# HalfSummer11/CAPTRA

Hardware: AMD Instinct MI355X
Metric: tracked frames/sec (4096-pt clouds) (higher is better)
Workload: dtype f32; 1 GPU; NOCS-REAL275-shaped rigid category 'bottle' (1 part, symmetric), 4096 pts/frame, batch=32 trajectories per GPU, fp32 (BASELINE.json configs[1]); points=4096, trajectories_per_gpu=32, distinct_clouds_per_gpu=32, parallelism=dp1 (trajectory-sharded, RCCL all-gather of poses), weights=seeded default_rng(7), real architecture (3.96 M params), physical-regime plants

## Files before the change

captra_amd/csrc/sa_pipe.hip:

```cpp
#include "wave_mlp.h"

namespace {

constexpr int SP_POS = 128;

struct SpParams {
    int b, n, m, k;
    const float *v1pm;
    const float *xyz_cn;
    const float *new_xyz;
    const int *idx;
    const float *w1;
    const float *w2, *b2, *w3, *b3;
    float *out;
    int out_ctotal, co_off;
    unsigned long long *prof;
    int split;
    int *dyn;
};

#define SP_TICK(slot)                                                           \
    if (CAPTRA_PROF_ON(p.prof)) {                                                    \
        const unsigned long long t_now = __builtin_amdgcn_s_memtime();          \
        if (lane == 0 && sampled) atomicAdd(p.prof + (slot), t_now - t_last);   \
        t_last = t_now;                                                         \
    }

template <int NOUT>
__device__ __forceinline__ void sp_mid_unit(const f32x16 &acc, int t, int q, float (&hout)[NOUT]) {
    unsigned a[4];
#pragma unroll
    for (int i = 0; i < 4; ++i) {
        const int x = __float_as_int(acc[4 * q + i]);
        a[i] = (unsigned)(x > 0 ? x : 0);
    }
    const auto p01 = __builtin_amdgcn_permlane32_swap(a[0], a[1], false, false);
    const auto p23 = __builtin_amdgcn_permlane32_swap(a[2], a[3], false, false);
    const int k0 = 16 * t + 4 * q;
    if (k0 + 0 < NOUT) hout[k0 + 0] = __uint_as_float(p01[0]);
    if (k0 + 1 < NOUT) hout[k0 + 1] = __uint_as_float(p23[0]);
    if (k0 + 2 < NOUT) hout[k0 + 2] = __uint_as_float(p01[1]);
    if (k0 + 3 < NOUT) hout[k0 + 3] = __uint_as_float(p23[1]);
}

struct SpMaxState {
    int w[8];
    int u[2];
};

__device__ __forceinline__ void sp_max_stage_a(const f32x16 &acc, SpMaxState &st, int lane) {
    const bool b0 = lane & 1;
#pragma unroll
    for (int i = 0; i < 8; ++i) {
        const int x0 = __float_as_int(acc[2 * i]), x1 = __float_as_int(acc[2 * i + 1]);
        const int own = b0 ? x1 : x0, oth = b0 ? x0 : x1;
        st.w[i] = imax_dpp<0xB1>(own, oth);
    }
}

__device__ __forceinline__ void sp_max_stage_bc(SpMaxState &st, int lane) {
    const bool b1 = lane & 2, b2 = lane & 4;
    int v[4];
#pragma unroll
    for (int j = 0; j < 4; ++j) {
        const int own = b1 ? st.w[2 * j + 1] : st.w[2 * j], oth = b1 ? st.w[2 * j] : st.w[2 * j + 1];
        v[j] = imax_dpp<0x4E>(own, oth);
    }
#pragma unroll
    for (int m = 0; m < 2; ++m) {
        const int own = b2 ? v[2 * m + 1] : v[2 * m], oth = b2 ? v[2 * m] : v[2 * m + 1];
        const int p = dpp_keep<0x104, 0xF, 0x5>(own, oth);
        const int q = dpp_keep<0x114, 0xF, 0xA>(p, oth);
        st.u[m] = imax(own, q);
    }
}

__device__ __forceinline__ void sp_max_stage_d(const SpMaxState &st, int &zr) {
    const int lane = (int)(threadIdx.x & 63);
    const bool b3 = lane & 8;
    const int own = b3 ? st.u[1] : st.u[0], oth = b3 ? st.u[0] : st.u[1];
    zr = imax(zr, imax_dpp<0x128>(own, oth));
}

template <int COUT, bool LAST, int NPARTS, int NOUT, int NZ>
__device__ __forceinline__ void sp_epi_part(const f32x16 (&acc)[2], int ps, int c, float (&hout)[NOUT], int (&zrun)[NZ],
                                            SpMaxState (&mst)[2], int lane) {
    constexpr int NT = (COUT + 31) / 32;
    if constexpr (LAST) {
#pragma unroll
        for (int u = 0; u < 6; ++u)
            if (u * NPARTS / 6 == c && 2 * ps + u / 3 < NT) {
                const int tm = u / 3;
                if (u % 3 == 0) sp_max_stage_a(acc[tm], mst[tm], lane);
                else if (u % 3 == 1) sp_max_stage_bc(mst[tm], lane);
                else sp_max_stage_d(mst[tm], zrun[2 * ps + tm < NZ ? 2 * ps + tm : 0]);
            }
    } else {
#pragma unroll
        for (int u = 0; u < 8; ++u)
            if (u * NPARTS / 8 == c && 2 * ps + (u >> 2) < NT) sp_mid_unit<NOUT>(acc[u >> 2], 2 * ps + (u >> 2), u & 3, hout);
    }
}


template <int CIN, int COUT, bool LAST, int START, int NIN, int NOUT, int NZ, typename Next, typename Side>
__device__ __forceinline__ void sp_layer(const float *wt, const float *bias_lds, const float (&hin)[NIN], float (&hout)[NOUT],
                                         float (&s)[3][16], int (&zrun)[NZ], int lane, Next next, Side side) {
    using S = SwShape<CIN, COUT>;
    static_assert(NIN >= S::KST, "input operand array too small");
    const __amdgpu_buffer_rsrc_t rsrc = sw_frag_rsrc<CIN, COUT>(wt);
    const int voff = lane * 16;
    f32x16 acc[2][2];
    SpMaxState mst[2];
    static_assert(!LAST || S::NSETS >= 6 || S::NPASS == 1, "the deferred max needs its six units in distinct steps, in order");
#pragma unroll
    for (int g = 0; g < S::STEPS; ++g) {
        const int ps = g / S::NSETS, c = g % S::NSETS, pb = ps & 1;
        if (c == 0) {
#pragma unroll
            for (int tm = 0; tm < 2; ++tm)
                if (2 * ps + tm < S::NT) sw_bias_init(acc[pb][tm], bias_lds, 2 * ps + tm, lane);
        }
        if (g == 0 && S::STEPS > 1) sw_load_set<CIN, COUT>(s[(START + 1) % 3], rsrc, voff, 1 / S::NSETS, 1 % S::NSETS);
        if (g + 2 < S::STEPS) sw_load_set<CIN, COUT>(s[(START + g + 2) % 3], rsrc, voff, (g + 2) / S::NSETS, (g + 2) % S::NSETS);
        if (g + 2 == S::STEPS || (S::STEPS == 1 && g == 0)) next(s[(START + S::STEPS) % 3]);
        side(g);
        __builtin_amdgcn_sched_barrier(0);
#pragma unroll
        for (int j = 0; j < SW_KS; ++j)
#pragma unroll
            for (int tm = 0; tm < 2; ++tm) {
                const int kk = c * SW_KS + j;
                if (kk < S::KST && 2 * ps + tm < S::NT)
                    acc[pb][tm] = __builtin_amdgcn_mfma_f32_32x32x2f32(s[(START + g) % 3][tm * SW_KS + j], hin[kk], acc[pb][tm], 0, 0, 0);
            }
        if (ps > 0) {
            sp_epi_part<COUT, LAST, S::NSETS>(acc[pb ^ 1], ps - 1, c, hout, zrun, mst, lane);
#pragma unroll
            for (int i = 0; i < 2 * SW_KS; ++i) {
                __builtin_amdgcn_sched_group_barrier(0x008, 1, 0);
                __builtin_amdgcn_sched_group_barrier(0x002, 4, 0);
            }
        }
        __builtin_amdgcn_sched_barrier(0);
    }
    constexpr int LP = S::NPASS - 1;
#pragma unroll
    for (int c = 0; c < S::NSETS; ++c) sp_epi_part<COUT, LAST, S::NSETS>(acc[LP & 1], LP, c, hout, zrun, mst, lane);
}

template <int CF, int C1, int C2, int C3>
__device__ __forceinline__ void sp_body(const SpParams &p, const int blk, const int nblk) {
    using S1 = SwShape<CF + 3, C1>;
    using S2 = SwShape<C1, C2>;
    using S3 = SwShape<C2, C3>;
    constexpr int NT1 = S1::NT;
    static_assert(NT1 <= 4 && C1 % 32 == 0, "first-layer width");
    __shared__ __attribute__((aligned(16))) float bias_lds[2 * 256];
    const int tid = threadIdx.x, lane = tid & 63, half = lane >> 5;
    const int wave = __builtin_amdgcn_readfirstlane(tid >> 6);

    for (int e = tid; e < 2 * 256; e += 256) {
        const int c = e & 255;
        bias_lds[e] = e < 256 ? (c < pad128c(C2) ? p.b2[c] : 0.f) : (c < pad128c(C3) ? p.b3[c] : 0.f);
    }
    float at[2][NT1];
    {
        const __amdgpu_buffer_rsrc_t rw = __builtin_amdgcn_make_buffer_rsrc((void *)p.w1, 0, S1::KP * S1::LDW * 4, 0x00020000);
        const int voff_w = (half * S1::LDW + (lane & 31)) * 4;
#pragma unroll
        for (int jj = 0; jj < 2; ++jj)
#pragma unroll
            for (int t = 0; t < NT1; ++t)
                at[jj][t] = __builtin_bit_cast(float, __builtin_amdgcn_raw_buffer_load_b32(rw, voff_w, ((CF + 2 * jj) * S1::LDW + 32 * t) * 4, 0));
    }
    __syncthreads();

    const int nwaves = nblk * 4, gid = blk * 4 + wave;
    const int ncentres = p.b * p.m;
    const int nslices = p.k / 32;
    int id = 0;
    float bt[2] = {0.f, 0.f};
    float4 g4[NT1][4];
    auto load_id = [&](int c, int sl) { return p.idx[(size_t)c * p.k + sl * 32 + (lane & 31)]; };
    auto load_rest = [&](int c, int id_, float (&bt_)[2], float4 (&g_)[NT1][4]) {
        const int tb = c / p.m;
        const float *cp = p.new_xyz + (size_t)c * 3;
#pragma unroll
        for (int jj = 0; jj < 2; ++jj) {
            const int a = 2 * jj + half;
            bt_[jj] = a < 3 ? p.xyz_cn[((size_t)tb * 3 + a) * p.n + id_] - cp[a] : 0.f;
        }
        const float4 *vp = reinterpret_cast<const float4 *>(p.v1pm + ((size_t)tb * p.n + id_) * C1 + 4 * half);
#pragma unroll
        for (int t = 0; t < NT1; ++t)
#pragma unroll
            for (int q = 0; q < 4; ++q) g_[t][q] = vp[8 * t + 2 * q];
    };

    const bool sampled = blk % 16 == 0;
    unsigned long long t_last = CAPTRA_PROF_ON(p.prof) ? __builtin_amdgcn_s_memtime() : 0ull;
    float s[3][16];
    constexpr int START3 = S2::STEPS % 3;
    constexpr int NEXT2 = (START3 + S3::STEPS) % 3;
    int zrun[S3::NT];
    const bool split = p.split != 0;
    const int ssh = __builtin_ctz((unsigned)nslices);
    int task = gid;
    int c = split ? gid >> ssh : gid, sl = split ? gid & (nslices - 1) : 0;
    const bool dyn = p.dyn != nullptr && !split && nslices > 1;
    int dyn_raw = 0, c_next = gid + nwaves;
    if (dyn) {
        if (lane == 0) dyn_raw = atomicAdd(p.dyn, 1);
        c = __builtin_amdgcn_readfirstlane(dyn_raw);
    }
    if (c < ncentres) {
        sw_first_set<C1, C2>(s[NEXT2], p.w2, lane);
        id = load_id(c, sl);
        load_rest(c, id, bt, g4);
    }
    while (c < ncentres) {
        if (sl == 0 || split) {
#pragma unroll
            for (int t = 0; t < S3::NT; ++t) zrun[t] = 0;
        }
        const bool last_slice = split || sl + 1 == nslices;
        if (dyn) {
            if (sl == 0 && lane == 0) dyn_raw = atomicAdd(p.dyn, 1);
            if (last_slice) c_next = __builtin_amdgcn_readfirstlane(dyn_raw);
        } else {
            c_next = c + nwaves;
        }
        const int cn = split ? (task + nwaves) >> ssh : (last_slice ? c_next : c), sn = split ? (task + nwaves) & (nslices - 1) : (last_slice ? 0 : sl + 1);
        const bool has_next = cn < ncentres;
        int id_n = 0;

        float h1[S2::KST], h2[S3::KST], none[1];
        SP_TICK(0)
        if (NEXT2 != 0) {
#pragma unroll
            for (int i = 0; i < 16; ++i) s[0][i] = s[NEXT2][i];
        }
        {
            f32x16 acc[NT1];
#pragma unroll
            for (int t = 0; t < NT1; ++t)
#pragma unroll
                for (int q = 0; q < 4; ++q) {
                    acc[t][4 * q + 0] = g4[t][q].x; acc[t][4 * q + 1] = g4[t][q].y;
                    acc[t][4 * q + 2] = g4[t][q].z; acc[t][4 * q + 3] = g4[t][q].w;
                }
#pragma unroll
            for (int jj = 0; jj < 2; ++jj)
#pragma unroll
                for (int t = 0; t < NT1; ++t) acc[t] = __builtin_amdgcn_mfma_f32_32x32x2f32(at[jj][t], bt[jj], acc[t], 0, 0, 0);
#pragma unroll
            for (int t = 0; t < NT1; ++t) sw_mid_epilogue<S2::KST>(acc[t], t, h1);
        }
        __builtin_amdgcn_sched_barrier(0);
        SP_TICK(1)
        sp_layer<C1, C2, false, 0>(p.w2, bias_lds, h1, h2, s, zrun, lane,
                                   [&](float (&dst)[16]) { sw_first_set<C2, C3>(dst, p.w3, lane); },
                                   [&](int g) { if (g == 1 && has_next) id_n = load_id(cn, sn); });
        SP_TICK(2)
        sp_layer<C2, C3, true, START3>(p.w3, bias_lds + 256, h2, none, s, zrun, lane,
                                       [&](float (&dst)[16]) { sw_first_set<C1, C2>(dst, p.w2, lane); },
                                       [&](int g) { if (g == 2 && has_next) load_rest(cn, id_n, bt, g4); });
        id = id_n;
        SP_TICK(3)
        if (CAPTRA_PROF_ON(p.prof) && lane == 0 && sampled) atomicAdd(p.prof + 9, 1ull);
        if (last_slice) {
            const int tb = c / p.m, centre = c - tb * p.m;
            const int r = lane & 15;
            const int row0 = 8 * (r >> 2) + (r & 3) + 4 * half;
            float *op = p.out + ((size_t)tb * p.out_ctotal + p.co_off + row0) * p.m + centre;
#pragma unroll
            for (int t = 0; t < S3::NT; ++t) {
                const float v = sw_bfly_finish(zrun[t]);
                if ((lane & 16) == 0 && 32 * t + row0 < C3) {
                    if (split) atomicMax(reinterpret_cast<int *>(op + (size_t)32 * t * p.m), __float_as_int(v));
                    else op[(size_t)32 * t * p.m] = v;
                }
            }
            SP_TICK(4)
        }
        c = cn; sl = sn; task += nwaves;
    }
}


template <int CF, int C1, int C2, int C3>
__global__ __launch_bounds__(256) __attribute__((amdgpu_waves_per_eu(1, 1))) void sa_wave_pipe_kernel(SpParams p) {
    sp_body<CF, C1, C2, C3>(p, (int)blockIdx.x, (int)gridDim.x);
}

struct Sp2Params { SpParams s[2]; int g0; };
__global__ __launch_bounds__(256) __attribute__((amdgpu_waves_per_eu(1, 1))) void sa_wave_pipe2_kernel(Sp2Params q) {
    const int blk = (int)blockIdx.x;
    if (blk < q.g0) sp_body<320, 128, 128, 256>(q.s[0], blk, q.g0);
    else sp_body<320, 128, 196, 256>(q.s[1], blk - q.g0, (int)gridDim.x - q.g0);
}

}

extern unsigned long long *captra_sa_prof_ptr();
extern int captra_sa_split_knob();
extern int *captra_sa_dyn_slot(const captra_launch_opts *o, hipStream_t stream);

struct SpRecord { SpParams q; unsigned grid; int code; };
struct SpCollect { SpRecord rec[2]; int n; };
void captra_sp_collect_init(void *buf, size_t bytes) {
    static_assert(sizeof(SpCollect) <= 1024, "SlCollect::sp (sa_fused.hip) holds an SpCollect");
    if (buf != nullptr && bytes >= sizeof(SpCollect)) static_cast<SpCollect *>(buf)->n = 0;
}
int captra_sp_collect_flush(void *buf, hipStream_t s) {
    SpCollect &c = *static_cast<SpCollect *>(buf);
    const int n = c.n;
    c.n = 0;
    if (n == 2 && c.rec[0].code == 0 && c.rec[1].code == 1 && c.rec[0].q.dyn == nullptr && c.rec[1].q.dyn == nullptr) {
        Sp2Params q2;
        q2.s[0] = c.rec[0].q; q2.s[1] = c.rec[1].q; q2.g0 = (int)c.rec[0].grid;
        CAPTRA_LAUNCH("sa_scale_fused", sa_wave_pipe2_kernel, dim3(c.rec[0].grid + c.rec[1].grid), dim3(256), 0, s, q2);
        return captra_last_error();
    }
    for (int i = 0; i < n; ++i) {
        if (c.rec[i].code == 0) { CAPTRA_LAUNCH("sa_scale_fused", (sa_wave_pipe_kernel<320, 128, 128, 256>), dim3(c.rec[i].grid), dim3(256), 0, s, c.rec[i].q); }
        else { CAPTRA_LAUNCH("sa_scale_fused", (sa_wave_pipe_kernel<320, 128, 196, 256>), dim3(c.rec[i].grid), dim3(256), 0, s, c.rec[i].q); }
    }
    return captra_last_error();
}

int captra_sa_scale_pre_pm_impl(int b, int n, int m, int k, int cfeat, int c1, int c2, int c3, const float *v1pm,
                                const float *xyz_cn, const float *new_xyz, const int *idx, const float *w1,
                                const float *w2, const float *b2, const float *w3, const float *b3, float *out,
                                int out_ctotal, int co_off, const captra_launch_opts *opts, void *spbuf, captra_stream_t stream) {
    SpCollect *col = static_cast<SpCollect *>(spbuf);
    if (b < 0 || n < 1 || m < 0 || k < 1 || cfeat < 1 || c1 < 1 || c2 < 1 || c3 < 1 || v1pm == nullptr) return -1;
    if (out_ctotal < co_off + c3 || co_off < 0) return -1;
    if (k % 32 != 0 || 128 % k != 0) return -2;
    const long long L = (long long)m * k;
    if (L % SP_POS != 0 || (long long)c1 * n * 4 >= (1ll << 31) || (long long)b * L >= (1ll << 31)) return -2;
    if (b == 0 || m == 0) return 0;
    SpParams q;
    q.b = b; q.n = n; q.m = m; q.k = k; q.v1pm = v1pm; q.xyz_cn = xyz_cn; q.new_xyz = new_xyz; q.idx = idx;
    q.w1 = w1; q.w2 = w2; q.b2 = b2; q.w3 = w3; q.b3 = b3; q.out = out; q.out_ctotal = out_ctotal; q.co_off = co_off;
    q.prof = captra_sa_prof_ptr();
    const int cus = captra_free_cus(opts);
    const long long centres = (long long)b * m;
    if (centres >= (1ll << 30)) return -2;
    const int split_knob = captra_sa_split_knob();
    q.split = (split_knob != 0 && k > 32 && (split_knob == 2 || centres < 4ll * cus)) ? 1 : 0;
    const long long wgs = ((q.split ? centres * (k / 32) : centres) + 3) / 4;
    const unsigned grid = (unsigned)(wgs < cus ? wgs : cus);
    q.dyn = (!q.split && k > 32 && wgs > 1 && col == nullptr) ? captra_sa_dyn_slot(opts, (hipStream_t)stream) : nullptr;
    if (q.split && !(opts != nullptr && opts->sa_prezeroed)) {
        if (b <= 8 && ((size_t)c3 * m * 4) % 16 == 0 && (reinterpret_cast<uintptr_t>(out + (size_t)co_off * m) & 15) == 0 && ((size_t)out_ctotal * m * 4) % 16 == 0) {
            for (int bb = 0; bb < b; ++bb) (void)captra_zero_async(out + ((size_t)bb * out_ctotal + co_off) * m, (size_t)c3 * m * 4, (hipStream_t)stream);
        } else {
            (void)hipMemset2DAsync(out + (size_t)co_off * m, (size_t)out_ctotal * m * 4, 0, (size_t)c3 * m * 4, b, (hipStream_t)stream);
        }
    }
#define SPP_CASE(CF_, C1_, C2_, C3_)                                                                                  \
    if (cfeat == CF_ && c1 == C1_ && c2 == C2_ && c3 == C3_) {                                                        \
        auto kern = sa_wave_pipe_kernel<CF_, C1_, C2_, C3_>;                                                          \
        if (col != nullptr && col->n < 2) {                                                                           \
            col->rec[col->n].q = q; col->rec[col->n].grid = grid; col->rec[col->n].code = (C2_ == 128 ? 0 : 1);       \
            ++col->n;                                                                                                 \
            return 0;                                                                                                 \
        }                                                                                                             \
        CAPTRA_LAUNCH("sa_scale_fused", kern, dim3(grid), dim3(256), 0, (hipStream_t)stream, q);                       \
        return captra_last_error();                                                                                   \
    }
    SPP_CASE(320, 128, 128, 256)
    SPP_CASE(320, 128, 196, 256)
#undef SPP_CASE
    return -2;
}

extern "C" int captra_sa_scale_pre_pm_ex(int b, int n, int m, int k, int cfeat, int c1, int c2, int c3, const float *v1pm,
                                         const float *xyz_cn, const float *new_xyz, const int *idx, const float *w1,
                                         const float *w2, const float *b2, const float *w3, const float *b3, float *out,
                                         int out_ctotal, int co_off, const captra_launch_opts *opts, captra_stream_t stream) {
    return captra_sa_scale_pre_pm_impl(b, n, m, k, cfeat, c1, c2, c3, v1pm, xyz_cn, new_xyz, idx, w1, w2, b2, w3, b3, out, out_ctotal, co_off, opts, nullptr, stream);
}
extern "C" int captra_sa_scale_pre_pm(int b, int n, int m, int k, int cfeat, int c1, int c2, int c3, const float *v1pm,
                                      const float *xyz_cn, const float *new_xyz, const int *idx, const float *w1,
                                      const float *w2, const float *b2, const float *w3, const float *b3, float *out,
                                      int out_ctotal, int co_off, captra_stream_t stream) {
    return captra_sa_scale_pre_pm_impl(b, n, m, k, cfeat, c1, c2, c3, v1pm, xyz_cn, new_xyz, idx, w1, w2, b2, w3, b3, out, out_ctotal, co_off, nullptr, nullptr, stream);
}
```

Before: 5891 frames/s.

## Compute layer-2 remainder channels with VALU FMAs instead of an extra MFMA tile

When the second MLP layer width leaves four channels past a multiple of 32, those four channels are now computed with scalar FMAs. Their weights are staged in LDS and h1 is exchanged across half-waves with permlane32 swaps. This avoids running a mostly empty 32-wide MFMA tile for them. The FMAs are interleaved into the MFMA schedule through an extra callback and adjusted sched_group_barrier counts. This adds VALU work, LDS traffic and register pressure, and only takes effect when C2 % 32 == 4.

```diff
diff --git a/captra_amd/csrc/sa_pipe.hip b/captra_amd/csrc/sa_pipe.hip
--- a/captra_amd/csrc/sa_pipe.hip
+++ b/captra_amd/csrc/sa_pipe.hip
@@ -103,9 +103,18 @@
 }
 
 
-template <int CIN, int COUT, bool LAST, int START, int NIN, int NOUT, int NZ, typename Next, typename Side>
+template <int NV>
+__device__ __forceinline__ void sp_interleave() {
+#pragma unroll
+    for (int i = 0; i < 2 * SW_KS; ++i) {
+        __builtin_amdgcn_sched_group_barrier(0x008, 1, 0);
+        __builtin_amdgcn_sched_group_barrier(0x002, NV, 0);
+    }
+}
+
+template <int CIN, int COUT, bool LAST, int START, int XSTEPS, int XV, int NIN, int NOUT, int NZ, typename Next, typename Side, typename Extra>
 __device__ __forceinline__ void sp_layer(const float *wt, const float *bias_lds, const float (&hin)[NIN], float (&hout)[NOUT],
-                                         float (&s)[3][16], int (&zrun)[NZ], int lane, Next next, Side side) {
+                                         float (&s)[3][16], int (&zrun)[NZ], int lane, Next next, Side side, Extra extra) {
     using S = SwShape<CIN, COUT>;
     static_assert(NIN >= S::KST, "input operand array too small");
     const __amdgpu_buffer_rsrc_t rsrc = sw_frag_rsrc<CIN, COUT>(wt);
@@ -134,14 +143,11 @@
                 if (kk < S::KST && 2 * ps + tm < S::NT)
                     acc[pb][tm] = __builtin_amdgcn_mfma_f32_32x32x2f32(s[(START + g) % 3][tm * SW_KS + j], hin[kk], acc[pb][tm], 0, 0, 0);
             }
-        if (ps > 0) {
-            sp_epi_part<COUT, LAST, S::NSETS>(acc[pb ^ 1], ps - 1, c, hout, zrun, mst, lane);
-#pragma unroll
-            for (int i = 0; i < 2 * SW_KS; ++i) {
-                __builtin_amdgcn_sched_group_barrier(0x008, 1, 0);
-                __builtin_amdgcn_sched_group_barrier(0x002, 4, 0);
-            }
-        }
+        if (g < XSTEPS) extra(g);
+        if (ps > 0) sp_epi_part<COUT, LAST, S::NSETS>(acc[pb ^ 1], ps - 1, c, hout, zrun, mst, lane);
+        if (ps > 0 && g < XSTEPS) sp_interleave<4 + XV>();
+        else if (ps > 0) sp_interleave<4>();
+        else if (g < XSTEPS) sp_interleave<XV>();
         __builtin_amdgcn_sched_barrier(0);
     }
     constexpr int LP = S::NPASS - 1;
@@ -151,18 +157,25 @@
 
 template <int CF, int C1, int C2, int C3>
 __device__ __forceinline__ void sp_body(const SpParams &p, const int blk, const int nblk) {
+    constexpr bool REM = C2 % 32 == 4;
+    constexpr int C2M = REM ? C2 - 4 : C2;
     using S1 = SwShape<CF + 3, C1>;
-    using S2 = SwShape<C1, C2>;
+    using S2 = SwShape<C1, C2M>;
     using S3 = SwShape<C2, C3>;
     constexpr int NT1 = S1::NT;
     static_assert(NT1 <= 4 && C1 % 32 == 0, "first-layer width");
+    static_assert(pad128c(C2M) == pad128c(C2) && S2::KST % SW_KS == 0, "layer-2 shape");
     __shared__ __attribute__((aligned(16))) float bias_lds[2 * 256];
+    __shared__ __attribute__((aligned(16))) float rem_w[REM ? 4 * C1 : 4];
     const int tid = threadIdx.x, lane = tid & 63, half = lane >> 5;
     const int wave = __builtin_amdgcn_readfirstlane(tid >> 6);
 
     for (int e = tid; e < 2 * 256; e += 256) {
         const int c = e & 255;
         bias_lds[e] = e < 256 ? (c < pad128c(C2) ? p.b2[c] : 0.f) : (c < pad128c(C3) ? p.b3[c] : 0.f);
+    }
+    if constexpr (REM) {
+        for (int e = tid; e < 4 * C1; e += 256) rem_w[(e & 3) * C1 + (e >> 2)] = p.w2[(size_t)(e >> 2) * S2::LDW + C2M + (e & 3)];
     }
     float at[2][NT1];
     {
@@ -257,15 +270,56 @@
 #pragma unroll
             for (int t = 0; t < NT1; ++t) sw_mid_epilogue<S2::KST>(acc[t], t, h1);
         }
+        float4 rw[2][REM ? SW_KS : 1];
+        float racc[2] = {0.f, 0.f};
+        auto rem_load = [&](int c) {
+            if constexpr (REM) {
+                const float4 *wp = reinterpret_cast<const float4 *>(rem_w + 2 * half * C1 + 2 * SW_KS * c);
+#pragma unroll
+                for (int i = 0; i < SW_KS; ++i) rw[c & 1][i] = wp[(i >> 2) * (C1 / 4) + (i & 3)];
+            }
+        };
+        auto rem_step = [&](int c) {
+            if constexpr (REM) {
+#pragma unroll
+                for (int j = 0; j < SW_KS; ++j) {
+                    const unsigned hb = __float_as_uint(h1[SW_KS * c + j]);
+                    const auto eo = __builtin_amdgcn_permlane32_swap(hb, hb, false, false);
+                    const float he = __uint_as_float(eo[0]), ho = __uint_as_float(eo[1]);
+#pragma unroll
+                    for (int r = 0; r < 2; ++r) {
+                        const float4 w4 = rw[c & 1][4 * r + (j >> 1)];
+                        racc[r] = __builtin_fmaf((j & 1) ? w4.z : w4.x, he, racc[r]);
+                        racc[r] = __builtin_fmaf((j & 1) ? w4.w : w4.y, ho, racc[r]);
+                    }
+                }
+                if (c == S2::NSETS - 1) {
+                    const int x0 = __float_as_int(racc[0]), x1 = __float_as_int(racc[1]);
+                    const auto pr = __builtin_amdgcn_permlane32_swap((unsigned)(x0 > 0 ? x0 : 0), (unsigned)(x1 > 0 ? x1 : 0), false, false);
+                    h2[C2M / 2] = __uint_as_float(pr[0]);
+                    h2[C2M / 2 + 1] = __uint_as_float(pr[1]);
+                }
+            }
+        };
+        if constexpr (REM) {
+            racc[0] = bias_lds[C2M + 2 * half];
+            racc[1] = bias_lds[C2M + 2 * half + 1];
+            rem_load(0);
+        }
         __builtin_amdgcn_sched_barrier(0);
         SP_TICK(1)
-        sp_layer<C1, C2, false, 0>(p.w2, bias_lds, h1, h2, s, zrun, lane,
+        sp_layer<C1, C2M, false, 0, REM ? S2::NSETS : 0, 5>(p.w2, bias_lds, h1, h2, s, zrun, lane,
                                    [&](float (&dst)[16]) { sw_first_set<C2, C3>(dst, p.w3, lane); },
-                                   [&](int g) { if (g == 1 && has_next) id_n = load_id(cn, sn); });
+                                   [&](int g) {
+                                       if (g == 1 && has_next) id_n = load_id(cn, sn);
+                                       if (g + 1 < S2::NSETS) rem_load(g + 1);
+                                   },
+                                   [&](int g) { rem_step(g); });
         SP_TICK(2)
-        sp_layer<C2, C3, true, START3>(p.w3, bias_lds + 256, h2, none, s, zrun, lane,
+        sp_layer<C2, C3, true, START3, 0, 0>(p.w3, bias_lds + 256, h2, none, s, zrun, lane,
                                        [&](float (&dst)[16]) { sw_first_set<C1, C2>(dst, p.w2, lane); },
-                                       [&](int g) { if (g == 2 && has_next) load_rest(cn, id_n, bt, g4); });
+                                       [&](int g) { if (g == 2 && has_next) load_rest(cn, id_n, bt, g4); },
+                                       [](int) {});
         id = id_n;
         SP_TICK(3)
         if (CAPTRA_PROF_ON(p.prof) && lane == 0 && sampled) atomicAdd(p.prof + 9, 1ull);
```

New measurement: 5963 frames/s, median of 6. 1.01x the previous value.
